# centreborelli/RVDD-release

Measured on AMD Instinct MI355X. Metric: frames/sec (whole job), recurrent video denoise+demosaic inference, higher is better.
Workload: dtype f32 (products as 3 split-f16 MFMAs, f32 accumulation)

## Files before the change

rvdd-release_amd/csrc/conv3x3h.hip:

```cpp
#include "rvdd_internal.h"

#include <type_traits>

namespace {

typedef _Float16 h8 __attribute__((ext_vector_type(8)));
typedef _Float16 h2 __attribute__((ext_vector_type(2)));
typedef __fp16 fp16x2 __attribute__((ext_vector_type(2)));
typedef unsigned int u32x4 __attribute__((ext_vector_type(4)));
typedef unsigned int u32x2 __attribute__((ext_vector_type(2)));
typedef __attribute__((address_space(3))) void lds_void;

constexpr int TW = 16;
constexpr int NTHREADS = 512;
constexpr int C8_PITCH = 16;

template <int CIN, int NGRP, int KS = 3, int MT = 3>
struct HGeo {
    static constexpr int PAD = KS / 2;
    static constexpr int TH = 16 / NGRP, IH = TH + KS - 1;
    static constexpr int IW = TW + KS - 1;
    static constexpr int NT = NTHREADS / NGRP;
    static constexpr int WPG = NT / 64;
    static constexpr int CMEM = CIN == 8 ? 16 : CIN;
    static constexpr int GPT = CIN / 8;
    static constexpr int NG = KS * KS * GPT;
    static constexpr int NCH = (NG + 3) / 4;
    static constexpr int HI = CIN * 2;
    static constexpr int S = CIN == 8 ? C8_PITCH : HI;
    static constexpr int PLANE = IH * IW * S;
    static constexpr int W_BYTES = NCH * MT * 2 * 1024;
    static constexpr int I_BYTES = 2 * PLANE;
    static constexpr int P_FLOATS = 48 + 3 * 48 + 4 + 8 + 4;
    static constexpr int LDS_BYTES = W_BYTES + NGRP * I_BYTES + P_FLOATS * 4;
    static constexpr int SEG = CIN / 4;
    static constexpr int ROWSEG = IW * SEG;
    static constexpr int RPR = NT / ROWSEG;
    static constexpr int NR = (IH + RPR - 1) / RPR;
    static constexpr int A_SPLIT = 7;
};

__device__ __forceinline__ f32x4 bload(__amdgpu_buffer_rsrc_t r, unsigned voff, int soff = 0) {
    return __builtin_bit_cast(f32x4, __builtin_amdgcn_raw_buffer_load_b128(r, voff, soff, 0));
}
__device__ __forceinline__ void bstore(__amdgpu_buffer_rsrc_t r, unsigned off, f32x4 v) {
    __builtin_amdgcn_raw_buffer_store_b128(__builtin_bit_cast(u32x4, v), r, off, 0, 0);
}

template <bool SCALED>
__device__ __forceinline__ void split4(f32x4 x, float sc, u32x2& hi, u32x2& lo) {
    if constexpr (SCALED) x = x * sc;
    const fp16x2 h01 = __builtin_amdgcn_cvt_pkrtz(x[0], x[1]);
    const fp16x2 h23 = __builtin_amdgcn_cvt_pkrtz(x[2], x[3]);
    const unsigned u01 = __builtin_bit_cast(unsigned, h01), u23 = __builtin_bit_cast(unsigned, h23);
    float r0, r1, r2, r3;
    asm("v_fma_mix_f32 %0, %1, -1.0, %2 op_sel_hi:[1,0,0]" : "=v"(r0) : "v"(u01), "v"(x[0]));
    asm("v_fma_mix_f32 %0, %1, -1.0, %2 op_sel:[1,0,0] op_sel_hi:[1,0,0]" : "=v"(r1) : "v"(u01), "v"(x[1]));
    asm("v_fma_mix_f32 %0, %1, -1.0, %2 op_sel_hi:[1,0,0]" : "=v"(r2) : "v"(u23), "v"(x[2]));
    asm("v_fma_mix_f32 %0, %1, -1.0, %2 op_sel:[1,0,0] op_sel_hi:[1,0,0]" : "=v"(r3) : "v"(u23), "v"(x[3]));
    const h2 l01 = {(_Float16)r0, (_Float16)r1};
    const h2 l23 = {(_Float16)r2, (_Float16)r3};
    hi = u32x2{u01, u23};
    lo = u32x2{__builtin_bit_cast(unsigned, l01), __builtin_bit_cast(unsigned, l23)};
}
struct TilePos {
    int b, y0, x0;
};

#ifdef RVDD_STAMPS
__device__ unsigned long long g_stamps[8 * 8];
#define STAMP_DECL unsigned long long st_acc[7] = {0, 0, 0, 0, 0, 0, 0}, st_t = __builtin_amdgcn_s_memtime(), st_n = 0
#define STAMP(i)                                                       \
    do {                                                               \
        const unsigned long long now_ = __builtin_amdgcn_s_memtime();  \
        st_acc[i] += now_ - st_t;                                      \
        st_t = now_;                                                   \
    } while (0)
#define STAMP_FLUSH                                                                        \
    do {                                                                                   \
        if ((threadIdx.x & 63) == 0) {                                                     \
            const int w_ = threadIdx.x >> 6;                                               \
            for (int i_ = 0; i_ < 7; ++i_) atomicAdd(&g_stamps[w_ * 8 + i_], st_acc[i_]);   \
            atomicAdd(&g_stamps[w_ * 8 + 7], st_n);                                        \
        }                                                                                  \
    } while (0)
#else
#define STAMP_DECL
// ... 248 lines not shown
    h8 Af[2][MT][2], Bf[2][2][2];
    auto read_frags = [&](int buf, int j) {
#pragma unroll
        for (int nt = 0; nt < 2; ++nt)
#pragma unroll
            for (int hl = 0; hl < 2; ++hl)
                Bf[buf][nt][hl] = __builtin_bit_cast(h8, *(lds_f4*)(boff[j] + nt * IW * G::S + hl * G::PLANE));
#pragma unroll
        for (int mt = 0; mt < MT; ++mt)
#pragma unroll
            for (int hl = 0; hl < 2; ++hl) {
                const int jj = j < G::A_SPLIT ? j : j - G::A_SPLIT;
                Af[buf][mt][hl] = __builtin_bit_cast(h8, *(lds_f4*)(abase[j < G::A_SPLIT ? 0 : 1] + ((jj * MT + mt) * 2 + hl) * 1024));
            }
    };

    const unsigned map_bytes = (unsigned)(a.H * a.W * kF * 4);
    constexpr bool SAME_OUT = CIN == 8;
    const unsigned out_bytes = SAME_OUT ? map_bytes : (unsigned)(a.Hout * a.Wout * kF * 4);

    float sc_nxt = 1.f, inv_cur = 1.f, inv_nxt = 1.f;
    float amx = 0.f;
    int amx_b = -1, pend_b = -1;
    unsigned* Rl = reinterpret_cast<unsigned*>(Pl + G::P_FLOATS - 12) + grp * G::WPG;
    auto amax_send = [&](int b) {
        unsigned t = lane < G::WPG ? Rl[lane] : 0u;
        t = amax_lines_max(t);
        if (lane == 0 && t)
            atomicMax(a.amax_out + (size_t)b * kAmaxSeqWords + (((MT == 3 ? blockIdx.x : blockIdx.x + blockIdx.y * 5u) * NGRP + grp) % kAmaxLines) * kAmaxLineWords, t);
    };
    typedef __attribute__((address_space(3))) unsigned lds_u32;
    lds_u32* gbar = (lds_u32*)(lds_u8*)(smem + G::W_BYTES + NGRP * G::I_BYTES + (G::P_FLOATS - 4) * 4) + grp;
    unsigned gcount = 0;
    auto gsync = [&]() {
        if constexpr (NGRP == 1) {
            __syncthreads();
        } else {
            gcount += G::WPG;
            asm volatile("s_waitcnt lgkmcnt(0)" ::: "memory");
            if (lane == 0) __hip_atomic_fetch_add(gbar, 1u, __ATOMIC_RELAXED, __HIP_MEMORY_SCOPE_WORKGROUP);
            while (__hip_atomic_load(gbar, __ATOMIC_RELAXED, __HIP_MEMORY_SCOPE_WORKGROUP) < gcount) __builtin_amdgcn_s_sleep(1);
            asm volatile("" ::: "memory");
        }
    };

    bool any_scaled = many_seqs;
    if (a.amax_in) {
        unsigned need = 0;
#pragma unroll
        for (int i = 0; i < 4; ++i) need |= (unsigned)amax_shift(amax_lines_max(ab_first[i]));
        any_scaled = any_scaled || need != 0;
    }

    t += grp * t_step;
    t_step *= NGRP;

    auto tile_loop = [&](auto scaled_tag) {
    constexpr bool SC = decltype(scaled_tag)::value;
    TilePos cur, nxt;
    locate(t, cur);
    {
        if constexpr (SC) {
            amax_fetch(cur.b, t < t_end);
            scale_from(ab_nxt, sc_nxt, inv_cur);
        }
        const Src q = source(cur, t < t_end);
        if constexpr (UPS) {
#pragma unroll
            for (int r0 = 0; r0 < UNR; ++r0) fetch_ups(q, r0);
#pragma unroll
            for (int r0 = 0; r0 < UNR; ++r0) interp_ups(q, r0, sc_nxt, scaled_tag);
        } else {
#pragma unroll
            for (int r0 = 0; r0 < G::NR; ++r0) fetch_round(q, r0);
#pragma unroll
            for (int r0 = 0; r0 < G::NR; ++r0) split4<SC>(pre[r0], sc_nxt, shi[r0], slo[r0]);
        }
        write_tile();
        asm volatile("s_waitcnt vmcnt(0)" ::: "memory");
        __syncthreads();
    }
    constexpr int NOUT = (EPI == EPI_POOL ? 1 : 2) * MT;
    f32x4 outv[NOUT];
    unsigned so_prev[2] = {0x80000000u, 0x80000000u};
    __amdgpu_buffer_rsrc_t orr_prev = __builtin_amdgcn_make_buffer_rsrc((void*)a.out, 0, 0, 0x00020000);
#pragma unroll
    for (int i = 0; i < NOUT; ++i) outv[i] = f32x4{0.f, 0.f, 0.f, 0.f};
    auto store_prev = [&](int i) {
        bstore(orr_prev, so_prev[EPI == EPI_POOL ? 0 : i / MT] + 64 * (mt0 + i % MT), outv[i]);
    };
    STAMP_DECL;
#pragma unroll 1
    while (t < t_end) {
        STAMP(0);
        gsync();
        STAMP(1);
        constexpr int SH = G::NCH >= 12 ? 1 : 0;
        constexpr int ST = G::NCH >= 14 ? (ACC_IN ? 1 : 7) : (G::NCH == 13 ? 6 : SH);
        constexpr int US = 3, UL = NGRP == 1 ? 4 : 3, UI = NGRP == 1 ? 5 : 3;
        Src qn;
        const int yy0 = cur.y0 + 2 * gw, xx = cur.x0 + n;
        unsigned po[2], so[2];
        f32x4 side[2][MT];
        __amdgpu_buffer_rsrc_t pr;
        auto addresses = [&]() {
            locate(t + t_step, nxt);
            qn = source(nxt, t + t_step < t_end);
            if constexpr (SC) amax_fetch(nxt.b, t + t_step < t_end);
        };
        auto addresses2 = [&]() {
#pragma unroll
            for (int nt = 0; nt < 2; ++nt) {
                const bool ok = yy0 + nt < a.H && xx < a.W;
                po[nt] = ok ? (unsigned)((((yy0 + nt) * a.W + xx) * kF + 4 * g) * 4) : 0x80000000u;
                so[nt] = SAME_OUT ? po[nt] : ok ? (unsigned)((((yy0 + nt + a.oy) * a.Wout + xx + a.ox) * kF + 4 * g) * 4) : 0x80000000u;
            }
            if constexpr (EPI == EPI_POOL) {
                const int pr_ = (cur.y0 >> 1) + gw, pc = xx >> 1;
                const bool ok = !(n & 1) && pr_ < a.Hout && pc < a.Wout;
                so[0] = ok ? (unsigned)(((pr_ * a.Wout + pc) * kF + 4 * g) * 4) : 0x80000000u;
            }
            pr = __builtin_amdgcn_make_buffer_rsrc((void*)((ACC_IN ? a.acc_in : a.out) + (size_t)cur.b * a.H * a.W * kF), 0, map_bytes,
                                                   0x00020000);
        };
        STAMP(2);

        f32x4 acc[2][MT];
        read_frags(0, 0);
#pragma unroll
        for (int j = 0; j < G::NCH; ++j) {
            const int cb = j & 1;
            if (j + 1 < G::NCH) read_frags(cb ^ 1, j + 1);
            if (j == SH) addresses();
            if (j == (G::NCH >= 14 ? 6 : SH)) addresses2();
            if (j >= ST && j - ST < NOUT) store_prev(j - ST);
            if constexpr (ACC_IN) {
                constexpr int SL = G::NCH >= 14 ? 7 : SH;
                if (j >= SL && j - SL < 2 * MT) side[(j - SL) / MT][(j - SL) % MT] = bload(pr, po[(j - SL) / MT], 64 * (mt0 + (j - SL) % MT));
            }
            if constexpr (SC) {
                if (j == (UPS ? SH + UL : G::NCH - 1 - (G::NR - 1) / 3)) scale_from(ab_nxt, sc_nxt, inv_nxt);
            }
            if constexpr (UPS) {
#pragma unroll
                for (int r0 = 0; r0 < UNR; ++r0) {
                    if (j == SH + US * r0) fetch_ups(qn, r0);
                    if (j == SH + UL + UI * r0) {
                        interp_ups(qn, r0, sc_nxt, scaled_tag);
#pragma unroll
                        for (int e = 0; e < 4; ++e) asm volatile("" : "+v"(ushi[r0][e]), "+v"(uslo[r0][e]));
                    }
                }
            } else {
                if (j >= SH && j - SH < G::NR) fetch_round(qn, j - SH);
#pragma unroll
                for (int r0 = 0; r0 < G::NR; ++r0)
                    if (j == G::NCH - 1 - (G::NR - 1 - r0) / 3) {
                        split4<SC>(pre[r0], sc_nxt, shi[r0], slo[r0]);
                        asm volatile("" : "+v"(shi[r0]), "+v"(slo[r0]));
                    }
            }
// ... 71 lines not shown
                for (int nt = 0; nt < 2; ++nt) {
                    float tq[3];
#pragma unroll
                    for (int c = 0; c < 3; ++c) {
                        float q = o3[nt][c];
                        q = lane_xor_add<16>(q);
                        q = lane_xor_add<32>(q);
                        tq[c] = q + Pl[4 * kF + c];
                    }
                    if (yy0 + nt < a.H && xx < a.W) m3 = fmaxf(m3, fmaxf(fmaxf(fabsf(tq[0]), fabsf(tq[1])), fabsf(tq[2])));
                    if (g == 0 && yy0 + nt < a.H && xx < a.W) {
                        const size_t pidx = (size_t)(yy0 + nt) * a.W + xx;
#pragma unroll
                        for (int c = 0; c < 3; ++c) a.out3_nchw[((size_t)cur.b * 3 + c) * hw + pidx] = tq[c];
                        if (a.out3_nhwc4)
                            reinterpret_cast<f32x4*>(a.out3_nhwc4)[(size_t)cur.b * hw + pidx] = f32x4{tq[0], tq[1], tq[2], 0.f};
                    }
                }
            }
        }
        if (a.amax_out) {
            if (cur.b != amx_b) {
                if (amx_b >= 0) {
                    const unsigned wm = wave_max_u32(__float_as_uint(amx));
                    if (lane == 0) Rl[gw] = wm;
                    pend_b = amx_b;
                }
                amx = 0.f;
                amx_b = cur.b;
            }
            float m0 = 0.f, m1 = 0.f;
#pragma unroll
            for (int i = 0; i < NOUT; ++i) {
                float& m = (EPI == EPI_POOL || i < MT) ? m0 : m1;
                asm("v_max3_f32 %0, %0, |%1|, |%2|" : "+v"(m) : "v"(outv[i][0]), "v"(outv[i][1]));
                asm("v_max3_f32 %0, %0, |%1|, |%2|" : "+v"(m) : "v"(outv[i][2]), "v"(outv[i][3]));
            }
            if (so[0] == 0x80000000u) m0 = 0.f;
            if (so[1] == 0x80000000u) m1 = 0.f;
            asm("v_max3_f32 %0, %0, %1, %2" : "+v"(amx) : "v"(m0), "v"(m1));
            amx = fmaxf(amx, m3);
        }
        so_prev[0] = so[0];
        so_prev[1] = so[1];
        orr_prev = __builtin_amdgcn_make_buffer_rsrc((void*)(a.out + (size_t)cur.b * (SAME_OUT ? a.H : a.Hout) * (SAME_OUT ? a.W : a.Wout) * kF), 0, out_bytes,
                                                     0x00020000);
        STAMP(4);
        gsync();
        STAMP(5);
        if (pend_b >= 0) {
            if (gw == 0) amax_send(pend_b);
            pend_b = -1;
        }
        write_tile();
        STAMP(6);
#ifdef RVDD_STAMPS
        ++st_n;
#endif
        t += t_step;
        cur = nxt;
        inv_cur = inv_nxt;
    }
#pragma unroll
    for (int j = 0; j < NOUT; ++j) store_prev(j);
    if (a.amax_out && amx_b >= 0) {
        gsync();
        const unsigned wm = wave_max_u32(__float_as_uint(amx));
        if (lane == 0) Rl[gw] = wm;
        gsync();
        if (gw == 0) amax_send(amx_b);
    }
    STAMP_FLUSH;
    };
    if (any_scaled) tile_loop(std::true_type{});
    else tile_loop(std::false_type{});
}

template <int CIN, int EPI, bool ACC_IN, bool UPS, int NGRP, int KS = 3, int MT = 3>
hipError_t launch_g(const ConvArgs& a0, hipStream_t s) {
    static std::atomic<uint64_t> attr_done{0};
    using G = HGeo<CIN, NGRP, KS, MT>;
    constexpr int TH = G::TH;
    void (*kern)(ConvArgs) = conv3x3h_kernel<CIN, EPI, ACC_IN, UPS, NGRP, KS, MT>;
    if (hipError_t e = allow_dynamic_lds(reinterpret_cast<const void*>(kern), G::LDS_BYTES, attr_done); e != hipSuccess) return e;
    ConvArgs a = a0;
    a.tiles_x = (a.W + TW - 1) / TW;
    a.tiles_y = (a.H + TH - 1) / TH;
    a.ntiles = a.B * a.tiles_x * a.tiles_y;
    const int cus = current_device_cus();
    const int want = (a.ntiles + NGRP - 1) / NGRP;
    const int grid = want < cus ? want : cus;
    hipLaunchKernelGGL(kern, dim3(grid, MT == 3 ? 1 : 3), dim3(NTHREADS), G::LDS_BYTES, s, a);
    return hipGetLastError();
}
bool cout_split_applies(const ConvArgs& a, bool enabled) {
    const int ntiles = a.B * ((a.W + TW - 1) / TW) * ((a.H + 15) / 16);
    return enabled && 3 * ntiles <= current_device_cus();
}
int g_conv3x3h_groups = 1;
template <int CIN, int EPI, bool ACC_IN, bool UPS = false>
hipError_t launch_h(const ConvArgs& a, hipStream_t s, bool cout_split) {
#ifdef RVDD_CONV_GROUPS2
    if (g_conv3x3h_groups == 2) return launch_g<CIN, EPI, ACC_IN, UPS, 2>(a, s);
#endif
    if constexpr (CIN == 48 && EPI != EPI_RELU_OUT3) {
        if (cout_split_applies(a, cout_split)) return launch_g<CIN, EPI, ACC_IN, UPS, 1, 3, 1>(a, s);
    }
    return launch_g<CIN, EPI, ACC_IN, UPS, 1>(a, s);
}

}

size_t conv3x3h_weight_bytes(int cin) { return cin == 48 ? HGeo<48, 1>::W_BYTES : HGeo<16, 1>::W_BYTES; }
size_t conv5x5h_weight_bytes(int cin) { return cin == 8 ? HGeo<8, 1, 5>::W_BYTES : HGeo<16, 1, 5>::W_BYTES; }

hipError_t launch_conv5x5h_c16(const ConvArgs& a, hipStream_t s) {
    if (a.B <= 0 || a.H <= 0 || a.W <= 0) return hipSuccess;
    if ((size_t)a.H * a.W * kF * 4 >= 0x80000000ull || a.acc_in || a.ups) return hipErrorInvalidValue;
    return launch_g<16, EPI_NONE, false, false, 1, 5>(a, s);
}
hipError_t launch_conv5x5h_c8(const ConvArgs& a, hipStream_t s) {
    if (a.B <= 0 || a.H <= 0 || a.W <= 0) return hipSuccess;
    if ((size_t)a.H * a.W * kF * 4 >= 0x80000000ull || a.acc_in || a.ups) return hipErrorInvalidValue;
    if (a.Hout != a.H || a.Wout != a.W || a.oy || a.ox) return hipErrorInvalidValue;
    return launch_g<8, EPI_NONE, false, false, 1, 5>(a, s);
}
void conv3x3h_set_groups(int g) { g_conv3x3h_groups = g == 1 ? 1 : 2; }

hipError_t launch_conv3x3h(const ConvArgs& a, int cin, int epi, hipStream_t s, bool cout_split) {
    if (a.B <= 0 || a.H <= 0 || a.W <= 0) return hipSuccess;
    if ((size_t)a.H * a.W * kF * 4 >= 0x80000000ull || (size_t)a.Hout * a.Wout * kF * 4 >= 0x80000000ull) return hipErrorInvalidValue;
    const bool acc = a.acc_in != nullptr;
    if (cin == 16) {
        if (acc || a.ups) return hipErrorInvalidValue;
        if (epi == EPI_NONE) return launch_h<16, EPI_NONE, false>(a, s, cout_split);
        if (epi == EPI_RELU) return launch_h<16, EPI_RELU, false>(a, s, cout_split);
        return hipErrorInvalidValue;
    }
    if (cin != 48) return hipErrorInvalidValue;
    if (a.ups) {
        if (acc || epi != EPI_RELU || (a.H & 1) || (a.W & 1)) return hipErrorInvalidValue;
        return launch_h<48, EPI_RELU, false, true>(a, s, cout_split);
    }
    switch (epi) {
        case EPI_NONE:
            return acc ? launch_h<48, EPI_NONE, true>(a, s, cout_split) : launch_h<48, EPI_NONE, false>(a, s, cout_split);
        case EPI_RELU:
            return acc ? launch_h<48, EPI_RELU, true>(a, s, cout_split) : launch_h<48, EPI_RELU, false>(a, s, cout_split);
        case EPI_POOL:
            return acc ? hipErrorInvalidValue : launch_h<48, EPI_POOL, false>(a, s, cout_split);
        case EPI_RELU_ADD2:
            return acc ? hipErrorInvalidValue : launch_h<48, EPI_RELU_ADD2, false>(a, s, cout_split);
        case EPI_RELU_OUT3:
            return acc ? hipErrorInvalidValue : launch_h<48, EPI_RELU_OUT3, false>(a, s, cout_split);
    }
    return hipErrorInvalidValue;
}
```

rvdd-release_amd/csrc/handle.hip:

```cpp
#include "runtime_internal.h"

namespace {

thread_local std::string g_create_error;

#define CONV_KERNEL_RANGE "rvdd_set_option: conv_kernel must be 0 (default), 1 (direct f32), 2 (winograd f32) or 4 (f32 by size)"

int conv_decode(const char* word, int32_t value) {
    static const struct { int sel; const char* word; } known[] = {
        {CONV_SPLIT16, nullptr}, {CONV_DIRECT, "direct"}, {CONV_WINO, "winograd"}, {CONV_F32, "f32"}};
    for (const auto& k : known)
        if (word ? (k.word && std::strcmp(word, k.word) == 0) : value == k.sel) return k.sel;
    return word ? CONV_SPLIT16 : -1;
}

void drop_graphs(rvdd_t* h) {
    for (auto& kv : h->graphs) {
        if (kv.second.exec) (void)hipGraphExecDestroy(kv.second.exec);
        if (kv.second.graph) (void)hipGraphDestroy(kv.second.graph);
    }
    h->graphs.clear();
}

bool graph_stream(rvdd_t* h) {
    if (h->gstream) return true;
    if (hipStreamCreateWithFlags(&h->gstream, hipStreamNonBlocking) != hipSuccess ||
        hipEventCreateWithFlags(&h->g_in, hipEventDisableTiming) != hipSuccess ||
        hipEventCreateWithFlags(&h->g_out, hipEventDisableTiming) != hipSuccess) {
        (void)hipGetLastError();
        if (h->gstream) (void)hipStreamDestroy(h->gstream);
        h->gstream = nullptr;
        return false;
    }
    return true;
}

int opt_graphs(rvdd_t* h, int32_t value) {
    h->opt.use_graphs = value && graph_stream(h);
    return RVDD_OK;
}
int opt_warp_raw(rvdd_t* h, int32_t value) {
    if (value && h->has_feat()) return fail(h, RVDD_ERR_ARG, "rvdd_set_option: warp_raw is not defined with feature recurrence (the reference fails there too)");
    h->opt.warp_raw = value;
    return RVDD_OK;
}
int opt_tvl1_async(rvdd_t* h, int32_t value) {
    if (!value && h->tvl1) {
        ENTER(h);
        HIPCHK(h, hipDeviceSynchronize());
        if (hipError_t e = tvl1_check(h->tvl1, nullptr); e != hipSuccess)
            return fail(h, RVDD_ERR_HIP, "rvdd_set_option(tvl1_async, 0): a pending asynchronous flow batch failed: %s", hipGetErrorString(e));
    }
    h->opt.tvl1_async = value;
    return RVDD_OK;
}
int opt_block_fp(rvdd_t* h, int32_t value) {
    h->opt.bfp = value;
    if (h->amax) {
        ENTER(h);
        HIPCHK(h, hipMemset(h->amax, 0, amax_bytes(h->cfg.batch, AMAX_SLOTS)));
    }
    return RVDD_OK;
}
int opt_conv_kernel(rvdd_t* h, int32_t value) {
    const int sel = conv_decode(nullptr, value);
    if (sel < 0) return fail(h, RVDD_ERR_ARG, "%s", CONV_KERNEL_RANGE);
    h->opt.conv = sel;
    return RVDD_OK;
}

#define RVDD_OPTIONS(F, X)                                                                                                       \
    F("no_warp", nullptr, no_warp, 0, 1, nullptr, nullptr)                                                                       \
    X("warp_raw", nullptr, warp_raw, 0, 1, nullptr, opt_warp_raw)                                                                \
    X("prev_noisy_frame", nullptr, prev_noisy, 0, 1, nullptr, nullptr)                                                           \
    X("conv_kernel", "RVDD_CONV", conv, 0, 4, CONV_KERNEL_RANGE, opt_conv_kernel)                                                \
    X("seq_major", "RVDD_SEQ_MAJOR", seq_major, 0, 1, "rvdd_set_option: seq_major must be 0 or 1", nullptr)                      \
    X("graphs", "RVDD_GRAPH", use_graphs, 0, 1, nullptr, opt_graphs)                                                             \
    X("fuse_upsample", "RVDD_FUSE_UPSAMPLE", fuse_upsample, 0, 1, nullptr, nullptr)                                              \
    X("next_split", "RVDD_NEXT_SPLIT", next_split, 0, 1, nullptr, nullptr)                                                       \
    X("next_pipe", "RVDD_NEXT_PIPE", next_pipe, 0, 1, nullptr, nullptr)                                                          \
    X("next_pool", "RVDD_NEXT_POOL", next_pool, 0, 1, nullptr, nullptr)                                                          \
    X("next_projfuse", "RVDD_NEXT_PROJFUSE", next_projfuse, 0, 1, nullptr, nullptr)                                              \
    X("tvl1_async", nullptr, tvl1_async, 0, 1, nullptr, opt_tvl1_async)                                                          \
    X("block_fp", "RVDD_BFP", bfp, 0, 1, nullptr, opt_block_fp)                                                                  \
    X("fuse_pre", "RVDD_FUSE_PRE", fuse_pre, 0, 1, nullptr, nullptr)                                                             \
    X("pre5_cin8", nullptr, pre5_cin8, 0, 1, nullptr, nullptr)                                                                   \
    X("cout_split", "RVDD_COUT_SPLIT", cout_split, 0, 1, nullptr, nullptr)                                                       \
    X("small_prestage", "RVDD_SMALL_PRESTAGE", small_prestage, 0, 1, nullptr, nullptr)                                           \
    X("warp48_pairs", nullptr, warp48_pairs, 0, 1, nullptr, nullptr)                                                             \
    X("bayer_pattern", nullptr, bayer, RVDD_BAYER_GBRG, RVDD_BAYER_BGGR,                                                         \
      "rvdd_set_option: bayer_pattern must be 0 (GBRG), 1 (GRBG), 2 (RGGB) or 3 (BGGR)", nullptr)                                \
    X("stream_reset_each", nullptr, stream_reset_each, 0, 1, nullptr, nullptr)                                                   \
    X("stream_flow_from_denoised", nullptr, stream_flow_from_denoised, 0, 1, nullptr, nullptr)                                   \
    X("stream_all_frames", nullptr, stream_all_frames, 0, 1, nullptr, nullptr)                                                   \
    X("stream_container", nullptr, stream_container, 0, 2,                                                                       \
      "rvdd_set_option: stream_container must be 0 (one number per sample), 1 (MIPI CSI-2) or 2 (MSB first)", nullptr)
struct OptRow {
    const char* name;
    const char* env;
    int Options::*field;
    int lo, hi;
    const char* range_msg;
    int (*hook)(rvdd_t*, int32_t);
};
#define OPT_ROW(name, env, field, lo, hi, msg, hook) {name, env, &Options::field, lo, hi, msg, hook},
const OptRow kOptions[] = {RVDD_OPTIONS(OPT_ROW, OPT_ROW)};
#define OPT_NAME_FIRST(name, ...) name
#define OPT_NAME(name, ...) ", " name
const char kUnknownOption[] = "rvdd_set_option: unknown option '%s' (known: " RVDD_OPTIONS(OPT_NAME_FIRST, OPT_NAME) ")";

int set_option_row(rvdd_t* h, const OptRow& row, int32_t value) {
    if (!row.range_msg) value = value != 0;
    else if (value < row.lo || value > row.hi) return fail(h, RVDD_ERR_ARG, "%s", row.range_msg);
    if (row.hook) return row.hook(h, value);
    h->opt.*row.field = value;
    return RVDD_OK;
}

struct KeySpec {
    std::string key;
    std::vector<int64_t> shape;
};

int convunet_cin(const rvdd_t* h, const std::string& name) {
    const bool feat = h->has_feat();
    if (name == "preprocessing_layer") return h->cin_real();
    if (name == "EncoderConvs.0.blocks.0.0") return feat ? 96 : h->cin_real();
    if (name.rfind("DecoderConvs.", 0) == 0 && name.find(".blocks.0.0") != std::string::npos) return 96;
    return 48;
}

std::vector<std::string> next_block_names(bool feat) {
    std::vector<std::string> n;
    for (int i = feat ? 0 : 1; i < NX_COUNT; ++i) n.push_back(kNxNames[i]);
    return n;
}

std::vector<KeySpec> expected_keys(const rvdd_t* h) {
    std::vector<KeySpec> k;
// ... 277 lines not shown
```

rvdd-release_amd/csrc/net_convunet.hip:

```cpp
#include "runtime_internal.h"

namespace {

std::vector<float> arrange_conv3x3(const HostTensor& t, int c0, int cn, int cin_pad) {
    const int cin_total = (int)t.shape[1];
    const int NJ = cin_pad / 16;
    std::vector<float> out((size_t)9 * NJ * 48 * 16, 0.f);
    for (int tap = 0; tap < 9; ++tap)
        for (int j = 0; j < NJ; ++j)
            for (int co = 0; co < 48; ++co)
                for (int g = 0; g < 4; ++g)
                    for (int i = 0; i < 4; ++i) {
                        const int c = 16 * j + 4 * g + i;
                        if (c >= cn) continue;
                        out[(((size_t)(tap * NJ + j) * 3 + co / 16) * 64 + g * 16 + co % 16) * 4 + i] =
                            t.data[(((size_t)co * cin_total + c0 + c) * 3 + tap / 3) * 3 + tap % 3];
                    }
    return out;
}

std::vector<float> arrange_wino3x3(const HostTensor& t, int c0, int nj = 3) {
    const int cin_total = (int)t.shape[1];
    const int nc = nj == 3 ? 48 : (cin_total < 16 ? cin_total : 16);
    static const double G[4][3] = {{1, 0, 0}, {0.5, 0.5, 0.5}, {0.5, -0.5, 0.5}, {0, 0, 1}};
// ... 151 lines not shown
    a.ntiles = a.B * a.tiles_x * a.tiles_y;
    const double px = (double)a.B * c.H * c.W;
    const double flops = 2.0 * 9.0 * L.cin_real[c.src] * 48.0 * px;
    double bytes = px * 4.0 * (L.cin_real[c.src] + (c.epi == EPI_POOL ? 12.0 : 48.0));
    if (c.acc_in) bytes += px * 192.0;
    if (c.epi == EPI_RELU_ADD2) bytes += px * 384.0;
    a.w3 = h->w_out;
    a.b3 = h->b_out;
    a.out3_nchw = c.out3_nchw ? c.out3_nchw + px_in * 3 : nullptr;
    a.out3_nhwc4 = c.out3_nhwc4 ? c.out3_nhwc4 + px_in * 4 : nullptr;
    a.amax_in = (c.amax_in >= 0 && h->opt.bfp) ? amax_words(h, c.amax_in, sub.b0) : nullptr;
    a.amax_out = (c.amax_out >= 0 && h->opt.bfp) ? amax_words(h, c.amax_out, sub.b0) : nullptr;
    const bool c16_ok = cin != 48 && !c.acc_in && (c.epi == EPI_NONE || c.epi == EPI_RELU);
    if (c.ups && !(cin == 48 && ((h->opt.split16() && L.wh[c.src]) || (L.wu[c.src] && wino_applies(h, run, c.H, c.W)))))
        return fail(h, RVDD_ERR_STATE, "run_conv: the fused upsample exists in the split-f16 and the Winograd kernels only");
    if (c.ups) bytes -= px * 4.0 * 36.0;
    if (h->opt.split16() && L.wh[c.src] && (cin == 48 || c16_ok)) {
        a.w = L.wh[c.src];
        a.wscale = L.wh_inv[c.src];
        Scope sc(h, s, c.ups ? "conv3x3h_kernel<48, 1, false, true>" : cin == 48 ? conv_name_h(c.epi, c.acc_in != nullptr)
                           : (c.epi == EPI_NONE ? "conv3x3h_kernel<16, 0, false, false>" : "conv3x3h_kernel<16, 1, false, false>"), flops, bytes);
        HIPCHK(h, launch_conv3x3h(a, cin == 48 ? 48 : 16, c.epi, s, h->opt.cout_split));
        return RVDD_OK;
    }
    if ((cin == 48 || c16_ok) && L.wu[c.src] && wino_applies(h, run, c.H, c.W)) {
        a.w = L.wu[c.src];
        Scope sc(h, s, c.ups ? "wino3x3_ups_kernel<1>" : cin == 48 ? wino_name(c.epi, c.acc_in != nullptr)
                                 : (c.epi == EPI_NONE ? "wino3x3_c16_kernel<0>" : "wino3x3_c16_kernel<1>"), flops, bytes);
        HIPCHK(h, launch_wino3x3(a, cin == 48 ? 48 : 16, c.epi, s));
        return RVDD_OK;
    }
    Scope sc(h, s, conv_name(cin, c.epi, c.acc_in != nullptr), flops, bytes);
    HIPCHK(h, launch_conv3x3(a, cin, c.epi, s, c.variant));
    return RVDD_OK;
}

int run_pre5(rvdd_t* h, const NetRun& run, const float* netin, float* part, hipStream_t s, Sub sub) {
    const int H = h->cfg.height, W = h->cfg.width;
    const size_t px0 = (size_t)sub.b0 * H * W;
    ConvArgs a{};
    a.in = netin + px0 * kNetInC;
    const bool c8 = h->opt.pre5_cin8 && h->pre5_w8;
    a.w = c8 ? h->pre5_w8 : h->pre5_w;
    a.wscale = c8 ? h->pre5_inv8 : h->pre5_inv;
    a.bias = h->pre5_b;
    a.out = part + px0 * kF;
    a.B = sub.nb;
    a.H = a.Hout = H;
    a.W = a.Wout = W;
    a.amax_in = h->opt.bfp ? amax_words(h, run.amax.base + AMAX_REL_NETIN, sub.b0) : nullptr;
    const double px = (double)sub.nb * H * W;
    {
        Scope sc(h, s, c8 ? "conv5x5h_kernel<8>" : "conv5x5h_kernel<16>", 2.0 * 25.0 * h->cin_real() * 48.0 * px, px * 4.0 * (h->cin_real() + 48.0));
        HIPCHK(h, c8 ? launch_conv5x5h_c8(a, s) : launch_conv5x5h_c16(a, s));
    }
    HIPCHK(h, launch_pre_border_fix(a.in, h->pre_w1, h->pre_b1, h->pre_w2, a.out, sub.nb, H, W, s));
    return RVDD_OK;
}

}

bool seq_major_on(const rvdd_t* h, int n) { return n > 1 && h->opt.seq_major == 1; }
bool pre5_fused(const rvdd_t* h) { return !h->is_next() && h->has_feat() && h->opt.fuse_pre && h->opt.split16() && h->pre5_w; }

int finalize_convunet(rvdd_t* h) {
    for (const auto& n : convunet_conv_names(h->has_feat())) {
        const HostTensor& wt = h->staged.at(n + ".weight");
        Conv3 L;
        const int cin = (int)wt.shape[1];
        if (cin == 96) {
            L.nsrc = 2;
            for (int sidx = 0; sidx < 2; ++sidx) {
                L.cin_real[sidx] = 48;
                L.cin_pad[sidx] = 48;
                RC(upload(h, &L.w[sidx], arrange_conv3x3(wt, 48 * sidx, 48, 48)));
                RC(upload(h, &L.wu[sidx], arrange_wino3x3(wt, 48 * sidx)));
                RC(upload(h, &L.wh[sidx], arrange_conv3x3h(wt, 48 * sidx, &L.wh_inv[sidx])));
            }
        } else {
            L.nsrc = 1;
            L.cin_real[0] = cin;
            L.cin_pad[0] = cin == 48 ? 48 : kNetInC;
            RC(upload(h, &L.w[0], arrange_conv3x3(wt, 0, cin, L.cin_pad[0])));
            RC(upload(h, &L.wu[0], cin == 48 ? arrange_wino3x3(wt, 0) : arrange_wino3x3(wt, 0, 1)));
            RC(upload(h, &L.wh[0], arrange_conv3x3h(wt, 0, &L.wh_inv[0], cin == 48 ? 48 : 16)));
        }
        RC(upload(h, &L.bias, h->staged.at(n + ".bias").data));
        for (int li = 0; li < CU_COUNT; ++li)
            if (n == kCuNames[li]) h->cu[li] = L;
    }
    RC(upload(h, &h->w_out, h->staged.at("PostConvs.1.weight").data));
    RC(upload(h, &h->b_out, h->staged.at("PostConvs.1.bias").data));
    if (h->has_feat()) RC(compose_pre_enc0(h));
    return RVDD_OK;
}

int run_convunet(rvdd_t* h, NetRun& run, const float* netin, const float* featw, float* feat_dst, float* out_nchw,
                 float* out_nhwc4, hipStream_t s) {
    const bool feat = h->has_feat();
    const int B = run.n;
    Level* lv = h->lv;
    const Conv3* cu = h->cu;
    auto conv = [&](int layer, const float* in, int from, float* out, int lvl, int epi, Sub sub) {
        ConvCall c;
        c.in = in; c.out = out; c.H = lv[lvl].H; c.W = lv[lvl].W; c.epi = epi;
        c.amax_in = from; c.amax_out = amax_layer(run, layer);
        return run_conv(h, run, cu[layer], c, s, sub);
// ... 139 lines not shown
```

rvdd-release_amd/csrc/runtime_internal.h:

```cpp
#pragma once
#include "../../include/rvdd.h"
#include "rvdd_internal.h"

#include <cmath>
#include <cstdarg>
#include <cstdio>
#include <cstdlib>
#include <cstring>
#include <map>
#include <string>
#include <vector>

struct HostTensor {
    std::vector<int64_t> shape;
    std::vector<float> data;
};

struct Conv3 {
    int nsrc = 0;
    int cin_real[2] = {0, 0};
    int cin_pad[2] = {0, 0};
    float* w[2] = {nullptr, nullptr};
    float* wu[2] = {nullptr, nullptr};
    float* wh[2] = {nullptr, nullptr};
// ... 50 lines not shown
    "DecoderConvs.2.blocks.0.0", "DecoderConvs.2.blocks.1.0", "PostConvs.0.0"};
constexpr int cu_enc(int level, int j) { return level == 0 ? CU_ENC0_0 + j : CU_ENC1_0 + 3 * (level - 1) + j; }
constexpr int cu_down(int i) { return CU_DOWN0 + 3 * i; }
constexpr int cu_up(int i) { return CU_UP0 + 3 * i; }
constexpr int cu_dec(int i, int j) { return CU_DEC0_0 + 3 * i + j; }
enum { AMAX_REL_NETIN = CU_COUNT, AMAX_REL_FWDFEAT, AMAX_NREG };
enum { AMAX_FEAT0 = 3 * AMAX_NREG, AMAX_SLOTS = AMAX_FEAT0 + 3 };

enum NxBlock {
    NX_PRE, NX_ENC0_0, NX_ENC0_1, NX_DOWN0, NX_ENC1_0, NX_ENC1_1, NX_DOWN1, NX_ENC2_0, NX_ENC2_1, NX_DOWN2, NX_ENC3_0,
    NX_ENC3_1, NX_BOT0, NX_BOT1, NX_UP0, NX_DEC0_0, NX_DEC0_1, NX_UP1, NX_DEC1_0, NX_DEC1_1, NX_UP2, NX_DEC2_0, NX_DEC2_1,
    NX_POST0, NX_POST1, NX_COUNT
};
inline const char* const kNxNames[NX_COUNT] = {
    "preprocessing_layer.blocks.0", "encoder_convs.0.blocks.0", "encoder_convs.0.blocks.1", "encoder_downs.0.postconv",
    "encoder_convs.1.blocks.0", "encoder_convs.1.blocks.1", "encoder_downs.1.postconv", "encoder_convs.2.blocks.0",
    "encoder_convs.2.blocks.1", "encoder_downs.2.postconv", "encoder_convs.3.blocks.0", "encoder_convs.3.blocks.1",
    "bottleneck.blocks.0", "bottleneck.blocks.1", "decoder_ups.0.postconv", "decoder_convs.0.blocks.0",
    "decoder_convs.0.blocks.1", "decoder_ups.1.postconv", "decoder_convs.1.blocks.0", "decoder_convs.1.blocks.1",
    "decoder_ups.2.postconv", "decoder_convs.2.blocks.0", "decoder_convs.2.blocks.1", "postprocessing.0.blocks.0",
    "postprocessing.0.blocks.1"};
constexpr int nx_enc(int level, int j) { return level == 0 ? NX_ENC0_0 + j : NX_ENC1_0 + 3 * (level - 1) + j; }
constexpr int nx_down(int i) { return NX_DOWN0 + 3 * i; }
constexpr int nx_up(int i) { return NX_UP0 + 3 * i; }
constexpr int nx_dec(int i, int j) { return NX_DEC0_0 + 3 * i + j; }

struct Level {
    int H = 0, W = 0;
    float* t[3] = {nullptr, nullptr, nullptr};
    float* skip = nullptr;
    float* part = nullptr;
};

enum ConvSel {
    CONV_SPLIT16 = 0,
    CONV_DIRECT = 1,
    CONV_WINO = 2,
    CONV_F32 = 4
};

struct Options {
    int no_warp = 0;
    int warp_raw = 0;
    int prev_noisy = 0;
    int bayer = 0;
    int conv = CONV_SPLIT16;
    int bfp = 1;
    int seq_major = 0;
    int fuse_upsample = 1;
    int cout_split = 1;
    int small_prestage = 1;
    int fuse_pre = 1;
    int pre5_cin8 = 1;
    int warp48_pairs = 0;
    int next_split = 1;
    int next_pipe = 1;
    int next_pool = 1;
    int next_projfuse = 1;
    int tvl1_async = 0;
    int stream_reset_each = 0;
    int stream_flow_from_denoised = 0;
    int stream_all_frames = 0;
    int stream_container = 0;
    int use_graphs = 0;

    bool split16() const { return conv == CONV_SPLIT16; }
    bool wino_allowed() const { return conv != CONV_DIRECT; }
    bool wino_forced() const { return conv == CONV_WINO; }
};

struct rvdd_handle {
    rvdd_cfg cfg{};
    std::string err;
    bool finalized = false;
    uint64_t reset_marks = 0;
    uint64_t undef_mask = 0;
    Options opt;
    bool serpentine = false;
    std::map<std::string, HostTensor> staged;
    std::vector<void*> allocs;

    Conv3 cu[CU_COUNT];
    float* pre5_w = nullptr;
    float pre5_inv = 1.f;
    float* pre5_b = nullptr;
    float* pre5_w8 = nullptr;
    float pre5_inv8 = 1.f;
    float* pre_w1 = nullptr;
    float* pre_b1 = nullptr;
    float* pre_w2 = nullptr;
    float* w_out = nullptr;
    float* b_out = nullptr;
    NextBlk nx[NX_COUNT];

    Level lv[4];
    float* netin = nullptr;
    float* lastden4 = nullptr;
    float* next4 = nullptr;
    float* green = nullptr;
    float* featw = nullptr;
    float* lastfeat = nullptr;
    unsigned* amax = nullptr;
    int step_ctr = 0;
    double* loss_batch = nullptr;
    size_t loss_batch_cap = 0;
    float* scratch = nullptr;
// ... 218 lines not shown
```

rvdd-release_amd/csrc/rvdd_internal.h:

```cpp
#pragma once
#include <hip/hip_runtime.h>
#include <stdint.h>

#include <atomic>

typedef float f32x4 __attribute__((ext_vector_type(4)));

constexpr int kF = 48;
constexpr int kNetInC = 16;

inline hipError_t allow_dynamic_lds(const void* kern, size_t bytes, std::atomic<uint64_t>& done) {
    int dev = 0;
    hipError_t e = hipGetDevice(&dev);
    if (e != hipSuccess) return e;
    const uint64_t bit = 1ull << (dev & 63);
    if (done.load(std::memory_order_acquire) & bit) return hipSuccess;
    e = hipFuncSetAttribute(kern, hipFuncAttributeMaxDynamicSharedMemorySize, (int)bytes);
    if (e == hipSuccess) done.fetch_or(bit, std::memory_order_release);
    return e;
}
inline int current_device_cus() {
    static std::atomic<int> cache[64];
    int dev = 0;
    if (hipGetDevice(&dev) != hipSuccess) return 256;
// ... 73 lines not shown
__device__ __forceinline__ float lane_xor_add(float v) {
    float a, b;
    lane_xor_pair<MASK>(v, a, b);
    return a + b;
}
template <int MASK>
__device__ __forceinline__ float lane_xor_max(float v) {
    float a, b;
    lane_xor_pair<MASK>(v, a, b);
    return fmaxf(a, b);
}
__device__ __forceinline__ unsigned wave_max_u32(unsigned v) {
    v = max(v, (unsigned)__builtin_amdgcn_update_dpp(0, (int)v, 0x111, 0xf, 0xf, true));
    v = max(v, (unsigned)__builtin_amdgcn_update_dpp(0, (int)v, 0x112, 0xf, 0xf, true));
    v = max(v, (unsigned)__builtin_amdgcn_update_dpp(0, (int)v, 0x114, 0xf, 0xf, true));
    v = max(v, (unsigned)__builtin_amdgcn_update_dpp(0, (int)v, 0x118, 0xf, 0xf, true));
    v = max(v, (unsigned)__builtin_amdgcn_update_dpp(0, (int)v, 0x142, 0xa, 0xf, true));
    v = max(v, (unsigned)__builtin_amdgcn_update_dpp(0, (int)v, 0x143, 0xc, 0xf, true));
    return (unsigned)__builtin_amdgcn_readlane((int)v, 63);
}
__device__ __forceinline__ unsigned amax_lines_max(unsigned v) {
    v = max(v, (unsigned)__builtin_amdgcn_update_dpp(0, (int)v, 0x111, 0xf, 0xf, true));
    v = max(v, (unsigned)__builtin_amdgcn_update_dpp(0, (int)v, 0x112, 0xf, 0xf, true));
    v = max(v, (unsigned)__builtin_amdgcn_update_dpp(0, (int)v, 0x114, 0xf, 0xf, true));
    v = max(v, (unsigned)__builtin_amdgcn_update_dpp(0, (int)v, 0x118, 0xf, 0xf, true));
    return (unsigned)__builtin_amdgcn_readlane((int)v, 15);
}
__device__ __forceinline__ void amax_commit_block(unsigned* words, int b, unsigned spread, float m, unsigned* red) {
    const unsigned mx = wave_max_u32(__float_as_uint(m));
    const int wave = threadIdx.x >> 6, nw = (blockDim.x + 63) >> 6;
    if ((threadIdx.x & 63) == 0) red[wave] = mx;
    __syncthreads();
    if (threadIdx.x == 0) {
        unsigned t = red[0];
        for (int i = 1; i < nw; ++i) t = max(t, red[i]);
        if (t) atomicMax(words + (size_t)b * kAmaxSeqWords + (spread % kAmaxLines) * kAmaxLineWords, t);
    }
}
__device__ __forceinline__ float absmax4(float m, f32x4 v) {
    return fmaxf(fmaxf(m, fmaxf(fabsf(v[0]), fabsf(v[1]))), fmaxf(fabsf(v[2]), fabsf(v[3])));
}
__device__ __forceinline__ bool seq_latched(unsigned long long mask, int b) {
    return mask == ~0ull || (b < 64 && ((mask >> b) & 1ull));
}
#endif

hipError_t launch_conv3x3(const ConvArgs& a, int cin, int epi, hipStream_t s, int variant = 0);
size_t conv3x3_weight_floats(int cin);
hipError_t launch_wino3x3(const ConvArgs& a, int cin, int epi, hipStream_t s);
size_t wino3x3_weight_floats();
hipError_t launch_conv3x3h(const ConvArgs& a, int cin, int epi, hipStream_t s, bool cout_split = true);
size_t conv3x3h_weight_bytes(int cin);
hipError_t launch_conv5x5h_c16(const ConvArgs& a, hipStream_t s);
hipError_t launch_conv5x5h_c8(const ConvArgs& a, hipStream_t s);
size_t conv5x5h_weight_bytes(int cin);
void conv3x3h_set_groups(int g);

hipError_t launch_pre_border_fix(const float* netin, const float* w1, const float* b1, const float* w2, float* part, int B, int H, int W,
                                 hipStream_t s);
hipError_t launch_relu_part(const float* part, float* out, int B, int64_t n, unsigned* words, hipStream_t s);
hipError_t launch_amax_reduce(const float* map, int B, int64_t hw_c, unsigned* words, hipStream_t s, int up = 0);

hipError_t launch_demosaic(const float* raw, float* green_scratch, float* out, int n, int h, int w,
                           int64_t bstride, int pstride, int cstride, hipStream_t s, int64_t raw_bstride, int bayer);
hipError_t launch_ha_green(const float* raw, float* green, int n, int h, int w, int64_t rbs, hipStream_t s, int bayer);
hipError_t launch_remosaick4(const float* rgb4, float* raw, int B, int H, int W, hipStream_t s, int bayer);

hipError_t launch_warp3(const float* src4, const float* flow_raw, float* dst, int dpstride, int B, int H, int W, hipStream_t s);
hipError_t launch_warp48(const float* src, const float* flow_raw, float* dst, int B, int H, int W, hipStream_t s, int64_t flow_bstride = 0,
                         bool pairs = false);
hipError_t launch_warp48_proj(const float* src, const float* flow_raw, float* dst, int B, int H, int W, const float* frag,
                              int inv_e, const float* bias, hipStream_t s, int64_t flow_bstride = 0);
hipError_t launch_warp_nchw(const float* x, const float* flow, float* y, int n, int c, int H, int W, hipStream_t s);
hipError_t launch_upsample_flow(const float* t, float* out, int nc, int h, int w, float mul, hipStream_t s);

hipError_t launch_netin(const float* raw_cur, float* green_scratch, const float* prev4, const float* flow_prev, const float* next4,
                        const float* flow_next, float* netin, int B, int h, int w, hipStream_t s, int64_t raw_bstride,
                        int64_t flow_bstride, const float* proj_w16, const float* proj_b, float* proj_out, int bayer);
hipError_t launch_netin_bound(const float* raw_a, const float* raw_b, const float* raw_c, int B, int h, int w, int64_t raw_bstride,
                              const unsigned* prev_words, unsigned* words, hipStream_t s, unsigned* zero_a = nullptr, size_t zero_na = 0,
                              unsigned* zero_b = nullptr, size_t zero_nb = 0, unsigned long long latch = ~0ull);
bool netin_small_applies(int B, int h, int w, bool future, bool enabled = true);
bool netin_tiled_applies(int h, int w, bool future, bool enabled = true);
hipError_t launch_netin_small(const float* raw_cur, const float* raw_prev, const float* prev4, const float* flow_prev, float* netin, int B,
                              int h, int w, int64_t raw_bstride, int64_t flow_bstride, const unsigned* prev_words, unsigned* words,
                              hipStream_t s, unsigned* zero_a, size_t zero_na, unsigned* zero_b, size_t zero_nb,
                              unsigned long long latch, int bayer);

hipError_t launch_upsample2x(const float* in, float* out, int B, int h, int w, int Hout, int Wout, int oy, int ox, bool align_corners, hipStream_t s);
hipError_t launch_maxpool2(const float* in, float* out, int B, int H, int W, hipStream_t s);
hipError_t launch_nchw_to_nhwc(const float* in, float* out, int B, int C, int H, int W, int Cpad, hipStream_t s);
hipError_t launch_nhwc_to_nchw(const float* in, float* out, int B, int C, int H, int W, int Cpad, hipStream_t s);
hipError_t launch_conv1x1_out(const float* feat, const float* w3x48, const float* b3, float* out_nchw,
                              float* out_nhwc4, int B, int H, int W, hipStream_t s);
hipError_t launch_loss_reduce_batch(const float* a, const float* b, int nslices, int64_t n, double* partial, int nblk,
                                    double* result2, hipStream_t s);

hipError_t launch_latch_zero(unsigned long long mask, float* feat, int64_t feat_per_seq, unsigned* words, int nsets, int B, hipStream_t s);
constexpr int kMaxMovePairs = 32;
hipError_t launch_move_slots(const int* from, const int* to, int count, float* den, int64_t den_per_seq, float* feat, int64_t feat_per_seq,
                             unsigned* words, int nsets, int B, hipStream_t s);

struct NextBlockW {
    const float* proj_w;
    const float* proj_b;
    const float* dw_w;
    const float* dw_b;
// ... 109 lines not shown
```

Measured before the change: 785.0.

## Run 5x5 cin8 prestage conv with two groups and LDS tile work queue

Launches the 5x5 conv for the 8-channel prestage with two half-height thread groups per block (NGRP=2) by default, instead of one group. For two-group kernels, the fixed strided tile assignment becomes a dynamic work queue held in LDS: each group claims its next tile with an atomic counter. This is meant to improve latency hiding and balance work between the groups. It adds LDS atomics and more weight-load overhead per block, and it also changes the two-group 3x3 path.

```diff
diff --git a/rvdd-release_amd/csrc/conv3x3h.hip b/rvdd-release_amd/csrc/conv3x3h.hip
--- a/rvdd-release_amd/csrc/conv3x3h.hip
+++ b/rvdd-release_amd/csrc/conv3x3h.hip
@@ -32,7 +32,8 @@
     static constexpr int W_BYTES = NCH * MT * 2 * 1024;
     static constexpr int I_BYTES = 2 * PLANE;
     static constexpr int P_FLOATS = 48 + 3 * 48 + 4 + 8 + 4;
-    static constexpr int LDS_BYTES = W_BYTES + NGRP * I_BYTES + P_FLOATS * 4;
+    static constexpr int Q_WORDS = NGRP == 2 ? 4 : 0;
+    static constexpr int LDS_BYTES = W_BYTES + NGRP * I_BYTES + P_FLOATS * 4 + Q_WORDS * 4;
     static constexpr int SEG = CIN / 4;
     static constexpr int ROWSEG = IW * SEG;
     static constexpr int RPR = NT / ROWSEG;
@@ -387,6 +388,11 @@
         any_scaled = any_scaled || need != 0;
     }
 
+    const int t0 = t, t_step0 = t_step;
+    lds_u32* tq = (lds_u32*)(lds_u8*)(smem + G::W_BYTES + NGRP * G::I_BYTES + G::P_FLOATS * 4);
+    if constexpr (NGRP == 2) {
+        if (tid >= 484 && tid < 487) tq[tid - 484] = tid == 484 ? 2u * NGRP : (unsigned)(NGRP + tid - 485);
+    }
     t += grp * t_step;
     t_step *= NGRP;
 
@@ -430,6 +436,8 @@
         STAMP(0);
         gsync();
         STAMP(1);
+        int t_q = 0;
+        if constexpr (NGRP == 2) t_q = t0 + __builtin_amdgcn_readfirstlane((int)tq[1 + grp]) * t_step0;
         constexpr int SH = G::NCH >= 12 ? 1 : 0;
         constexpr int ST = G::NCH >= 14 ? (ACC_IN ? 1 : 7) : (G::NCH == 13 ? 6 : SH);
         constexpr int US = 3, UL = NGRP == 1 ? 4 : 3, UI = NGRP == 1 ? 5 : 3;
@@ -439,9 +447,10 @@
         f32x4 side[2][MT];
         __amdgpu_buffer_rsrc_t pr;
         auto addresses = [&]() {
-            locate(t + t_step, nxt);
-            qn = source(nxt, t + t_step < t_end);
-            if constexpr (SC) amax_fetch(nxt.b, t + t_step < t_end);
+            const int t_nxt = NGRP == 2 ? t_q : t + t_step;
+            locate(t_nxt, nxt);
+            qn = source(nxt, t_nxt < t_end);
+            if constexpr (SC) amax_fetch(nxt.b, t_nxt < t_end);
         };
         auto addresses2 = [&]() {
 #pragma unroll
@@ -619,12 +628,16 @@
             if (gw == 0) amax_send(pend_b);
             pend_b = -1;
         }
+        if constexpr (NGRP == 2) {
+            if (gw == 0 && lane == 0) tq[1 + grp] = __hip_atomic_fetch_add(tq, 1u, __ATOMIC_RELAXED, __HIP_MEMORY_SCOPE_WORKGROUP);
+        }
         write_tile();
         STAMP(6);
 #ifdef RVDD_STAMPS
         ++st_n;
 #endif
-        t += t_step;
+        if constexpr (NGRP == 2) t = t_q;
+        else t += t_step;
         cur = nxt;
         inv_cur = inv_nxt;
     }
@@ -664,6 +677,7 @@
     const int ntiles = a.B * ((a.W + TW - 1) / TW) * ((a.H + 15) / 16);
     return enabled && 3 * ntiles <= current_device_cus();
 }
+bool pre5_two_groups(const ConvArgs& a) { return (long long)a.B * ((a.W + TW - 1) / TW) * ((a.H + 7) / 8) >= 2; }
 int g_conv3x3h_groups = 1;
 template <int CIN, int EPI, bool ACC_IN, bool UPS = false>
 hipError_t launch_h(const ConvArgs& a, hipStream_t s, bool cout_split) {
@@ -686,10 +700,11 @@
     if ((size_t)a.H * a.W * kF * 4 >= 0x80000000ull || a.acc_in || a.ups) return hipErrorInvalidValue;
     return launch_g<16, EPI_NONE, false, false, 1, 5>(a, s);
 }
-hipError_t launch_conv5x5h_c8(const ConvArgs& a, hipStream_t s) {
+hipError_t launch_conv5x5h_c8(const ConvArgs& a, hipStream_t s, int groups) {
     if (a.B <= 0 || a.H <= 0 || a.W <= 0) return hipSuccess;
     if ((size_t)a.H * a.W * kF * 4 >= 0x80000000ull || a.acc_in || a.ups) return hipErrorInvalidValue;
     if (a.Hout != a.H || a.Wout != a.W || a.oy || a.ox) return hipErrorInvalidValue;
+    if (groups != 1 && pre5_two_groups(a)) return launch_g<8, EPI_NONE, false, false, 2, 5>(a, s);
     return launch_g<8, EPI_NONE, false, false, 1, 5>(a, s);
 }
 void conv3x3h_set_groups(int g) { g_conv3x3h_groups = g == 1 ? 1 : 2; }
diff --git a/rvdd-release_amd/csrc/handle.hip b/rvdd-release_amd/csrc/handle.hip
--- a/rvdd-release_amd/csrc/handle.hip
+++ b/rvdd-release_amd/csrc/handle.hip
@@ -66,6 +66,10 @@
     const int sel = conv_decode(nullptr, value);
     if (sel < 0) return fail(h, RVDD_ERR_ARG, "%s", CONV_KERNEL_RANGE);
     h->opt.conv = sel;
+    return RVDD_OK;
+}
+int opt_pre5_groups(rvdd_t* h, int32_t value) {
+    h->opt.pre5_groups = value == 1 ? 1 : 2;
     return RVDD_OK;
 }
 
@@ -85,6 +89,7 @@
     X("block_fp", "RVDD_BFP", bfp, 0, 1, nullptr, opt_block_fp)                                                                  \
     X("fuse_pre", "RVDD_FUSE_PRE", fuse_pre, 0, 1, nullptr, nullptr)                                                             \
     X("pre5_cin8", nullptr, pre5_cin8, 0, 1, nullptr, nullptr)                                                                   \
+    X("pre5_groups", nullptr, pre5_groups, 0, 2, "rvdd_set_option: pre5_groups must be 1 or 2 (0: the default, 2)", opt_pre5_groups)   \
     X("cout_split", "RVDD_COUT_SPLIT", cout_split, 0, 1, nullptr, nullptr)                                                       \
     X("small_prestage", "RVDD_SMALL_PRESTAGE", small_prestage, 0, 1, nullptr, nullptr)                                           \
     X("warp48_pairs", nullptr, warp48_pairs, 0, 1, nullptr, nullptr)                                                             \
diff --git a/rvdd-release_amd/csrc/net_convunet.hip b/rvdd-release_amd/csrc/net_convunet.hip
--- a/rvdd-release_amd/csrc/net_convunet.hip
+++ b/rvdd-release_amd/csrc/net_convunet.hip
@@ -227,7 +227,7 @@
     const double px = (double)sub.nb * H * W;
     {
         Scope sc(h, s, c8 ? "conv5x5h_kernel<8>" : "conv5x5h_kernel<16>", 2.0 * 25.0 * h->cin_real() * 48.0 * px, px * 4.0 * (h->cin_real() + 48.0));
-        HIPCHK(h, c8 ? launch_conv5x5h_c8(a, s) : launch_conv5x5h_c16(a, s));
+        HIPCHK(h, c8 ? launch_conv5x5h_c8(a, s, h->opt.pre5_groups) : launch_conv5x5h_c16(a, s));
     }
     HIPCHK(h, launch_pre_border_fix(a.in, h->pre_w1, h->pre_b1, h->pre_w2, a.out, sub.nb, H, W, s));
     return RVDD_OK;
diff --git a/rvdd-release_amd/csrc/runtime_internal.h b/rvdd-release_amd/csrc/runtime_internal.h
--- a/rvdd-release_amd/csrc/runtime_internal.h
+++ b/rvdd-release_amd/csrc/runtime_internal.h
@@ -126,6 +126,7 @@
     int small_prestage = 1;
     int fuse_pre = 1;
     int pre5_cin8 = 1;
+    int pre5_groups = 2;
     int warp48_pairs = 0;
     int next_split = 1;
     int next_pipe = 1;
diff --git a/rvdd-release_amd/csrc/rvdd_internal.h b/rvdd-release_amd/csrc/rvdd_internal.h
--- a/rvdd-release_amd/csrc/rvdd_internal.h
+++ b/rvdd-release_amd/csrc/rvdd_internal.h
@@ -149,7 +149,7 @@
 hipError_t launch_conv3x3h(const ConvArgs& a, int cin, int epi, hipStream_t s, bool cout_split = true);
 size_t conv3x3h_weight_bytes(int cin);
 hipError_t launch_conv5x5h_c16(const ConvArgs& a, hipStream_t s);
-hipError_t launch_conv5x5h_c8(const ConvArgs& a, hipStream_t s);
+hipError_t launch_conv5x5h_c8(const ConvArgs& a, hipStream_t s, int groups = 2);
 size_t conv5x5h_weight_bytes(int cin);
 void conv3x3h_set_groups(int g);
 
```

New measurement: 789.4, median of 6. Within noise of the previous version (+0.6%).
